# yhz0/SQLP

Hardware: AMD Instinct MI355X
Metric: stage-2 subproblems/sec + cut-gen HBM GB/s on STORM (higher is better)
Workload: dtype f64

## Files before the change

include/twosd_hip.h:

```cpp
#ifndef TWOSD_HIP_H
#define TWOSD_HIP_H

#include <stdint.h>

#ifdef __cplusplus
extern "C" {
#endif

typedef struct twosd_ctx twosd_ctx;

enum {
    TWOSD_OK = 0,
    TWOSD_E_ARG = -1,
    TWOSD_E_DEVICE = -2,
    TWOSD_E_STATE = -3,
    TWOSD_E_LP = -4,
    TWOSD_E_UNSUPPORTED = -5
};

enum { TWOSD_LP_OPTIMAL = 0, TWOSD_LP_INFEASIBLE = 1, TWOSD_LP_ITER_LIMIT = 2, TWOSD_LP_NUMERIC = 3 };

const char *twosd_last_error(void);

const char *twosd_version(void);
// ... 14 lines not shown
                         int index_base, int *m_lp, int *n_lp, int *n_bound_rows, int64_t *out_colptr,
                         int64_t *out_rowval, double *out_nzval, double *out_q, double *out_r, char *out_sense,
                         double *c0, int *col_src, double *col_sign, double *col_off, int *col_src2, int *box_col);

int twosd_set_random_positions(twosd_ctx *ctx, int k, const int *row, const int *col, int index_base);

int twosd_compute_basis(twosd_ctx *ctx, const double *x, const double *values);
int twosd_set_basis(twosd_ctx *ctx, const int *head);
int twosd_get_basis(twosd_ctx *ctx, int *head);

int twosd_pool_add_basis(twosd_ctx *ctx, const int *head, int *added);
int twosd_pool_build(twosd_ctx *ctx, int epi, const double *x, int first, int count, int max_pool,
                     int *pool_size);
int twosd_pool_build_candidates(twosd_ctx *ctx, int epi, const double *x, int first, int count, int level1,
                                int ncand);
int twosd_pool_refresh(twosd_ctx *ctx, int epi, const double *x, int first, int count, int max_pool,
                       int *pool_size);
int twosd_last_refresh_ms(twosd_ctx *ctx, double *ms5);

int twosd_refresh_train(twosd_ctx *ctx, int epi, const double *x, int first, int count, int *n_bases, double *box_lo,
                        double *box_hi);
int twosd_refresh_train_ex(twosd_ctx *ctx, int epi, const double *x, int first, int count, int kcap, int *n_bases,
                           int *n_optimal, double *box_lo, double *box_hi);
int twosd_refresh_cap_stats(twosd_ctx *ctx, int64_t *pivots_sum, int64_t *scenarios);
int twosd_training_cap(twosd_ctx *ctx, int64_t pivots_sum, int64_t scenarios, int *cap);
int twosd_select_refresh_bases(const uint64_t *keys, const int64_t *counts, const int64_t *reps, const int32_t *rank_of,
                               int n, int max_pool, int64_t *owner, int64_t *rep, int *npick);
int twosd_refresh_train_bases(twosd_ctx *ctx, uint64_t *keys, int *counts, int *reps);
int twosd_refresh_build_local(twosd_ctx *ctx, int n_own, const int *reps, int64_t *pack_bytes);
int twosd_refresh_pack(twosd_ctx *ctx, void *d_dst);
// ... 210 lines not shown
```

sqlp_amd/_lib.py:

```python
from __future__ import annotations

import ctypes as C
import os

_HERE = os.path.dirname(os.path.abspath(__file__))
LIB_PATH = os.path.join(_HERE, f"libtwosd_hip_{os.environ['TWOSD_LIB']}.so" if os.environ.get("TWOSD_LIB")
                        else "libtwosd_hip.so")

TWOSD_OK = 0
ERRORS = {-1: "TWOSD_E_ARG", -2: "TWOSD_E_DEVICE", -3: "TWOSD_E_STATE", -4: "TWOSD_E_LP",
          -5: "TWOSD_E_UNSUPPORTED"}
LP_OPTIMAL, LP_INFEASIBLE, LP_ITER_LIMIT, LP_NUMERIC = 0, 1, 2, 3

P = C.c_void_p
I = C.c_int
D = C.c_double
SIGNATURES = [
    ("twosd_last_error", C.c_char_p, []),
    ("twosd_version", C.c_char_p, []),
    ("twosd_create", I, [I, P]),
    ("twosd_destroy", I, [P]),
    ("twosd_set_template", I, [P, I, I, I, P, P, P, P, P, P, P, P, P, P, P, I]),
    ("twosd_lp_shape", I, [P, P, P, P]),
    ("twosd_canonical_form", I, [I, I, P, P, P, P, P, P, P, P, I, P, P, P, P, P, P, P, P, P, P, P, P, P, P, P]),
    ("twosd_set_random_positions", I, [P, I, P, P, I]),
    ("twosd_compute_basis", I, [P, P, P]),
    ("twosd_set_basis", I, [P, P]),
    ("twosd_get_basis", I, [P, P]),
    ("twosd_pool_add_basis", I, [P, P, P]),
    ("twosd_pool_build", I, [P, I, P, I, I, I, P]),
    ("twosd_pool_build_candidates", I, [P, I, P, I, I, I, I]),
    ("twosd_pool_refresh", I, [P, I, P, I, I, I, P]),
    ("twosd_last_refresh_ms", I, [P, P]),
    ("twosd_pool_size", I, [P, P]),
    ("twosd_pool_get", I, [P, I, P]),
    ("twosd_last_pool_picks", I, [P, I, P]),
    ("twosd_invalidate_x", I, [P]),
    ("twosd_epigraph_create", I, [P, P]),
    ("twosd_add_scenarios", I, [P, I, I, P, P]),
    ("twosd_epigraph_info", I, [P, I, P, P]),
    ("twosd_set_distributions", I, [P, I, P, P, P, P, P, P]),
    ("twosd_add_sampled_scenarios", I, [P, I, I, C.c_uint64, C.c_uint64, P]),
    ("twosd_get_scenarios", I, [P, I, I, I, P]),
    ("twosd_evaluate_sampled", I, [P, P, C.c_int64, C.c_int64, C.c_int64, C.c_uint64, P]),
    ("twosd_moments_merge", I, [P, P, P]),
    ("twosd_moments_of_values", I, [P, C.c_int64, P, P, P]),
# ... 142 lines not shown
```

sqlp_amd/csrc/lp_hyper.hip:

```cpp
#include <hip/hip_runtime.h>
#include <math.h>
#include <type_traits>
#include "twosd_internal.h"
#include "wave_ops.h"

namespace twosd {

#define HTOL_P 1e-9
#define HTOL_D 1e-9
#define HTOL_PIV 1e-9
#define HPI_ZERO 1e-12


#ifdef TWOSD_STAMPS
#define STAMP_DECL unsigned long long st_acc[10] = {0, 0, 0, 0, 0, 0, 0, 0, 0, 0}; \
    unsigned long long st_last = __builtin_amdgcn_s_memtime();
#define STAMP(i)                                                      \
    {                                                                 \
        const unsigned long long t_ = __builtin_amdgcn_s_memtime();   \
        st_acc[i] += t_ - st_last;                                    \
        st_last = t_;                                                 \
    }
#define STAMP_FLUSH                                                                         \
    if (lane == 0 && P.stamps)                                                              \
// ... 1035 lines not shown
    const int wid = __builtin_amdgcn_readfirstlane(threadIdx.x >> 6);
    const int s0 = blockIdx.x * kSelTile;
    const int ns = min(kSelTile, S.N - s0);
    const int sent = h_sel_sentinel(S.k);
    h_stage_sentinel(dvt, S.k);
    h_stage_pairs(dvt, S.dv, S.kcoef, S.k, ns, [&](int sl) { return s0 + sl; });
    if (threadIdx.x < kSelTile) sbest[threadIdx.x] = 0x7f800000u;
    __syncthreads();
    sel_f2 best = {INFINITY, INFINITY};
    int bpx = 0, bpy = 0;
    auto alive2 = [&](sel_f2 inf) {
        const float ox = __uint_as_float(__hip_atomic_load(&sbest[lane], __ATOMIC_RELAXED, __HIP_MEMORY_SCOPE_WORKGROUP));
        const float oy = __uint_as_float(__hip_atomic_load(&sbest[64 + lane], __ATOMIC_RELAXED, __HIP_MEMORY_SCOPE_WORKGROUP));
        return (inf.x < best.x && inf.x <= ox) || (inf.y < best.y && inf.y <= oy);
    };
    const int p_lo = (int)((long long)S.npool * blockIdx.y / gridDim.y), p_hi = (int)((long long)S.npool * (blockIdx.y + 1) / gridDim.y);
    bpx = bpy = p_lo;
    for (int p = p_lo + wid; p < p_hi; p += kSelWaves) {
        const sel_f2 inf = h_stream2(S.rec, S.sptr[p], S.send[p], S.cinf[p], S.cw, dvt2, sent, lane, alive2);
        if (inf.x < best.x) {
            best.x = inf.x;
            bpx = p;
            atomicMin(&sbest[lane], __float_as_uint(inf.x));
        }
        if (inf.y < best.y) {
            best.y = inf.y;
            bpy = p;
            atomicMin(&sbest[64 + lane], __float_as_uint(inf.y));
        }
    }
    bsum[wid][lane] = best.x; bidx[wid][lane] = bpx;
// ... 88 lines not shown
                const int cw = rci[w][sl];
                if (v < bk || (v == bk && cw >= 0 && (bc < 0 ? false : cw < bc))) { bk = v; bc = cw; }
            }
            const int s = S.order[t0 + sl];
            if (gridDim.y > 1) {
                S.pkey[(size_t)blockIdx.y * S.N + s] = bk;
                S.pci[(size_t)blockIdx.y * S.N + s] = bc;
            } else if (bc >= 0) {
                S.pick[s] = S.cand[(size_t)S.pick[s] * S.ncand + bc];
            }
        }
    }
}

__global__ void pool_select_merge_kernel(int N, int G, const float *__restrict__ pkey, const int *__restrict__ ppick, int *pick,
                                         float *key) {
    const int s = blockIdx.x * blockDim.x + threadIdx.x;
    if (s >= N) return;
    float b = pkey[s];
    int bp = ppick[s];
    for (int y = 1; y < G; ++y) {
        const float v = pkey[(size_t)y * N + s];
        const int p = ppick[(size_t)y * N + s];
        if (v < b || (v == b && p < bp)) { b = v; bp = p; }
    }
    pick[s] = bp;
    if (key) key[s] = b;
}
__global__ void pool_refine_merge_kernel(int N, int G, int ncand, const float *__restrict__ pkey, const int *__restrict__ pci,
                                         const int *__restrict__ cand, int *pick) {
    const int s = blockIdx.x * blockDim.x + threadIdx.x;
    if (s >= N) return;
    float bk = pkey[s];
    int bc = pci[s];
    for (int y = 1; y < G; ++y) {
        const float v = pkey[(size_t)y * N + s];
        const int c = pci[(size_t)y * N + s];
        if (v < bk || (v == bk && c >= 0 && (bc < 0 ? false : c < bc))) { bk = v; bc = c; }
    }
    if (bc >= 0) pick[s] = cand[(size_t)pick[s] * ncand + bc];
}

static int sel_split(int N, int items) {
    if (getenv("TWOSD_SEL_NOSPLIT")) return 1;
    const int nb = (N + kSelTile - 1) / kSelTile;
    int g = (1024 + nb - 1) / nb;
    g = std::min(g, std::max(1, items / kSelWaves));
    return std::max(1, std::min(g, 64));
}
int pool_select_split(int N, int npool) { return sel_split(N, npool); }
int pool_refine_split(int N, int ncand) { return sel_split(N, ncand); }

hipError_t launch_pool_refine(const PoolRefineParams &p, hipStream_t s) {
    if (p.N <= 0 || p.ncand <= 0) return hipSuccess;
    const int G = p.pkey ? pool_refine_split(p.N, p.ncand) : 1;
    hipLaunchKernelGGL(pool_refine_kernel, dim3((p.N + kSelTile - 1) / kSelTile, G), dim3(64 * kSelWaves), pool_select_lds_bytes(p.k), s, p);
    if (G > 1) hipLaunchKernelGGL(pool_refine_merge_kernel, dim3((p.N + 255) / 256), dim3(256), 0, s, p.N, G, p.ncand, p.pkey, p.pci, p.cand, p.pick);
    return hipGetLastError();
}

size_t pool_select_lds_bytes(int k) { return (size_t)4 * 65 * (kSelTile / 64) * (size_t)(std::max(k, 0) + 1); }

hipError_t launch_pool_select(const PoolSelParams &p, hipStream_t s) {
    if (p.N <= 0) return hipSuccess;
    const int nb = (p.N + kSelTile - 1) / kSelTile;
    const int G = p.pkey ? pool_select_split(p.N, p.npool) : 1;
    hipLaunchKernelGGL(pool_select_kernel, dim3(nb, G), dim3(64 * kSelWaves), pool_select_lds_bytes(p.k), s, p);
    if (G > 1) hipLaunchKernelGGL(pool_select_merge_kernel, dim3((p.N + 255) / 256), dim3(256), 0, s, p.N, G, p.pkey, p.ppick, p.pick, p.key);
    return hipGetLastError();
}

__global__ void __launch_bounds__(256) queue_records_kernel(int N, const int *__restrict__ order, const int *__restrict__ pick,
                                                           int2 *__restrict__ qrec) {
    const int q = blockIdx.x * blockDim.x + threadIdx.x;
    if (q >= N) return;
    const int s = order ? order[q] : q;
    qrec[q] = make_int2(s, pick ? pick[s] : 0);
}
hipError_t launch_queue_records(const int *order, const int *pick, int2 *qrec, int N, hipStream_t s) {
    if (N <= 0) return hipSuccess;
    hipLaunchKernelGGL(queue_records_kernel, dim3((N + 255) / 256), dim3(256), 0, s, N, order, pick, qrec);
    return hipGetLastError();
}
// ... 79 lines not shown
```

sqlp_amd/csrc/pool_refresh.hip:

```cpp
#include <hip/hip_runtime.h>
#include <algorithm>
#include <chrono>
#include <cmath>
#include <cstdio>
#include <cstdlib>
#include <cstring>
#include <vector>
#include "twosd_internal.h"
#include "twosd_ctx.h"

using namespace twosd;

using Clock = std::chrono::steady_clock;
static double ms_between(Clock::time_point a, Clock::time_point b) { return std::chrono::duration<double, std::milli>(b - a).count(); }


static const char *finish_composed(const twosd_ctx *c, PoolBasis &B) {
    const HostLP &L = c->L;
    pi0_from_rows(c, B);
    if (sparse_dual_infeasibility(L, B.head, B.pi0) > 1e-7) return "composed basis is not dual feasible";
    if (sparse_basis_residual(L, B.head, B.rptr, B.rcol, B.rval, 4) > 1e-8) return "composed B^{-1} inconsistent";
    return nullptr;
}

// ... 156 lines not shown
}

extern "C" int twosd_refresh_cap_stats(twosd_ctx *c, int64_t *pivots_sum, int64_t *scenarios) {
    if (!c) return fail(TWOSD_E_ARG, "refresh_cap_stats: NULL");
    if (pivots_sum) *pivots_sum = c->piv_ref_sum;
    if (scenarios) *scenarios = c->piv_ref_n;
    return TWOSD_OK;
}

extern "C" int twosd_set_refresh_kcap(twosd_ctx *c, int kcap) {
    if (!c) return fail(TWOSD_E_ARG, "set_refresh_kcap: NULL");
    c->train_kcap = kcap;
    return TWOSD_OK;
}

static int refresh_training(twosd_ctx *c, const double *x, const double *d_dv, int count, int kcap, bool retry, int *n_opt, bool dbg) {
    LpRun o;
    o.want_bkey = true;
    o.want_etas = true;
    o.want_head = true;
    o.kcap = kcap;
    int rc;
    if ((rc = run_lp(c, x, d_dv, count, o))) return rc;
    int opt = count;
    if (o.kcap > 0) {
        std::vector<int> st(count);
        HIPCHK(hipMemcpy(st.data(), c->d_status, sizeof(int) * count, hipMemcpyDeviceToHost));
        opt = (int)std::count(st.begin(), st.end(), (int)TWOSD_LP_OPTIMAL);
        if (retry && 2 * opt < count) {
            if (dbg) fprintf(stderr, "refresh training: %d of %d optimal under cap %d, solved again uncapped\n", opt, count, o.kcap);
            o.kcap = 0;
            if ((rc = run_lp(c, x, d_dv, count, o))) return rc;
        }
    }
    HIPCHK(hipStreamSynchronize(c->stream));
    unsigned long long used64 = 0;
    HIPCHK(hipMemcpy(&used64, c->d_eo_used, sizeof(used64), hipMemcpyDeviceToHost));
    if (used64 > c->eo_cap && used64 <= (unsigned long long)INT32_MAX) {
        if (dbg) fprintf(stderr, "refresh training: eta files of %llu entries past the arena of %zu, solved again\n", used64, c->eo_cap);
        c->eo_min_cap = (size_t)std::min<unsigned long long>(used64 + used64 / 8, INT32_MAX);
        if ((rc = run_lp(c, x, d_dv, count, o))) return rc;
    }
    c->last_train_opt = opt;
    if (n_opt) *n_opt = opt;
    return TWOSD_OK;
}

namespace {
struct RefreshFront {
    const EpiDevice *E = nullptr;
    const double *d_dv = nullptr;
    std::vector<int> reps, cnts;
// ... 36 lines not shown
        HIPCHK(hipMemcpy(F.reps.data(), d_list, sizeof(int) * U, hipMemcpyDeviceToHost));
        HIPCHK(hipMemcpy(F.cnts.data(), d_counts, sizeof(int) * U, hipMemcpyDeviceToHost));
    }
    F.t_bases = Clock::now();
    return TWOSD_OK;
}

extern "C" int twosd_pool_refresh(twosd_ctx *c, int epi, const double *x, int first, int count, int max_pool,
                                  int *pool_size) {
    const bool dbg = getenv("TWOSD_DEBUG") != nullptr;
    RefreshFront F;
    int rc;
    if ((rc = refresh_front(c, "pool_refresh", epi, x, first, count, max_pool >= 1, -1, true, nullptr, nullptr, dbg, F))) return rc;
    const int m = c->L.m, U = (int)F.reps.size();
    std::vector<int> ord(U);
    for (int a = 0; a < U; ++a) ord[a] = a;
    std::stable_sort(ord.begin(), ord.end(), [&](int a, int b) { return F.cnts[a] > F.cnts[b]; });
    const int R = std::min(U, max_pool - 1);
    std::vector<int> sel(R);
    for (int a = 0; a < R; ++a) sel[a] = F.reps[ord[a]];
    std::vector<PoolBasis> fresh;
    bool device_built = false;
    c->last_refresh_ms[1] = ms_between(F.t_trained, F.t_bases);
    c->last_refresh_ms[2] = c->last_refresh_ms[3] = 0.0;
    if (R > 0 && !getenv("TWOSD_REFRESH_HOST")) {
        if ((rc = c->d_refresh_sel.fit((size_t)R))) return rc;
        HIPCHK(hipMemcpyAsync(c->d_refresh_sel, sel.data(), sizeof(int) * R, hipMemcpyHostToDevice, c->stream));
        const int dev = refresh_build_device(c, R, dbg);
        if (dev < 0) return dev;
        device_built = dev == 0;
        c->last_refresh_ms[2] = ms_between(F.t_bases, Clock::now());
    }
// ... 336 lines not shown
```

sqlp_amd/csrc/pool_select.hip:

```cpp
#include <hip/hip_runtime.h>
#include <algorithm>
#include <cmath>
#include <cstdio>
#include <cstdlib>
#include <vector>
#include <chrono>
#include "twosd_internal.h"
#include "twosd_ctx.h"

using namespace twosd;

void twosd::reset_candidates(twosd_ctx *c) {
    c->pool_l1 = c->pool_ncand = 0;
    c->cand_pending = false;
    std::vector<int>().swap(c->cand_p1);
    std::vector<int>().swap(c->cand_pf);
}

int twosd::reserve_selection(twosd_ctx *c, int P, int records) {
    int rc;
    if ((rc = c->d_sel_code.fit(2 * (size_t)std::max(records, 1)))) return rc;
    if ((rc = c->d_sel_end.reserve((size_t)P)) || (rc = c->d_sel_cinf.reserve((size_t)P))) return rc;
    c->sel_cap_total = records;
    return TWOSD_OK;
// ... 316 lines not shown
            for (int p = 0; p < P; ++p) c->sel_nnz += end[p] - beg[p];
        }
    }
    c->prep_x.assign(x, x + n1);
    c->prep_valid = true;
    if (getenv("TWOSD_DEBUG")) {
        HIPCHK(hipStreamSynchronize(c->stream));
        fprintf(stderr, "prepare_x: P=%d %.3f ms (%lld selection records)\n", P,
                std::chrono::duration<double, std::milli>(std::chrono::steady_clock::now() - t_start).count(),
                (long long)c->sel_nnz);
    }
    return TWOSD_OK;
}

static int set_candidates(twosd_ctx *c, int level1, int ncand, int n, const int *p1, const int *pf) {
    std::vector<int> start(level1 + 1, 0);
    for (int s = 0; s < n; ++s)
        if (pf[s] != p1[s] && p1[s] >= 0 && p1[s] < level1) ++start[p1[s] + 1];
    for (int p = 0; p < level1; ++p) start[p + 1] += start[p];
    std::vector<int> fill(start.begin(), start.end() - 1), bucket(start[level1]);
    for (int s = 0; s < n; ++s)
        if (pf[s] != p1[s] && p1[s] >= 0 && p1[s] < level1) bucket[fill[p1[s]]++] = pf[s];
    std::vector<int> cand((size_t)level1 * ncand, -1);
    std::vector<std::pair<int, int>> v;
    for (int p = 0; p < level1; ++p) {
        int *b0 = bucket.data() + start[p], *b1 = bucket.data() + start[p + 1];
        if (b0 == b1) continue;
        std::sort(b0, b1);
        v.clear();
        for (int *a = b0; a < b1;) {
            int *b = a;
            while (b < b1 && *b == *a) ++b;
            v.push_back({-(int)(b - a), *a});
            a = b;
        }
        const size_t nk = std::min<size_t>(v.size(), ncand);
        std::partial_sort(v.begin(), v.begin() + nk, v.end());
        for (size_t i = 0; i < nk; ++i) cand[(size_t)p * ncand + i] = v[i].second;
    }
    if (getenv("TWOSD_DEBUG")) {
        int diff = 0, filled = 0;
        for (int s = 0; s < n; ++s) diff += pf[s] != p1[s];
        for (int v : cand) filled += v >= 0;
        fprintf(stderr, "pool candidates: P=%zu level1=%d: %d of %d training picks change, %d candidate slots filled\n",
                c->bp.bases.size(), level1, diff, n, filled);
    }
    int rc;
    int *h = c->stage[STG_CAND].reserve<int>(cand.size());
    if (!h) return fail(TWOSD_E_DEVICE, "pool candidates: pinned staging allocation failed");
    std::copy(cand.begin(), cand.end(), h);
    if ((rc = c->d_cand.reserve(cand.size()))) return rc;
    HIPCHK(hipMemcpyAsync(c->d_cand, h, sizeof(int) * cand.size(), hipMemcpyHostToDevice, c->stream));
    c->pool_l1 = level1;
    c->pool_ncand = ncand;
    c->cand_pending = false;
    return TWOSD_OK;
}

int twosd::select_pool(twosd_ctx *c, const double *d_dv, int N, int *d_pick, int npool_override) {
    const int P = (int)c->bp.bases.size();
    const bool two = npool_override <= 0 && c->pool_l1 > 0 && c->pool_l1 < P && c->pool_ncand > 0 && (c->d_cand || c->cand_pending);
    const int np1 = npool_override > 0 ? npool_override : two ? c->pool_l1 : P;
    int rc;
    size_t tb = 0, tb2 = 0;
    HIPCHK(sort_by_pool(d_pick, nullptr, N, P, nullptr, &tb, c->stream));
    HIPCHK(sort_by_pool(d_pick, nullptr, N, np1, nullptr, &tb2, c->stream));
    tb = std::max(tb, tb2);
    if ((size_t)N > c->d_order.cap || tb > c->d_sort_tmp.cap) {
        if ((rc = c->d_order.alloc((size_t)N)) || (rc = c->d_sort_tmp.alloc(tb))) return rc;
    }
    if (two && (rc = c->d_sel_key.fit((size_t)N))) return rc;
    const int g1 = pool_select_split(N, np1), g2 = two ? pool_refine_split(N, c->pool_ncand) : 1;
    const size_t pneed = (size_t)std::max(g1, g2) * N;
    if (std::max(g1, g2) > 1 && ((rc = c->d_sel_pkey.fit(pneed)) || (rc = c->d_sel_ppick.fit(pneed)))) return rc;
    PoolSelParams S{};
    S.N = N; S.k = c->k; S.npool = np1; S.dv = d_dv;
    S.kcoef = c->d_kcoef;
    S.cinf = c->d_sel_cinf; S.sptr = c->d_sel_ptr; S.send = c->d_sel_end; S.rec = reinterpret_cast<const int2 *>(c->d_sel_code.p);
    S.pick = d_pick;
    S.cw = c->sel_cw;
    S.key = two ? c->d_sel_key : nullptr;
    S.pkey = g1 > 1 ? c->d_sel_pkey : nullptr;
    S.ppick = g1 > 1 ? c->d_sel_ppick : nullptr;
    HIPCHK(launch_pool_select(S, c->stream));
    if (two && c->cand_pending &&
        (rc = set_candidates(c, c->cand_pl1, c->cand_pnc, (int)c->cand_p1.size(), c->cand_p1.data(), c->cand_pf.data())))
        return rc;
    if (two) {
        HIPCHK(sort_by_pool(d_pick, c->d_order, N, np1, c->d_sort_tmp, &tb, c->stream));
        PoolRefineParams Q{};
        Q.N = N; Q.k = c->k; Q.ncand = c->pool_ncand; Q.dv = d_dv; Q.kcoef = c->d_kcoef;
        Q.cinf = c->d_sel_cinf; Q.sptr = c->d_sel_ptr; Q.send = c->d_sel_end; Q.rec = S.rec;
        Q.order = c->d_order; Q.cand = c->d_cand; Q.pick = d_pick; Q.key = c->d_sel_key; Q.cw = c->sel_cw;
        Q.pkey = g2 > 1 ? c->d_sel_pkey : nullptr;
        Q.pci = g2 > 1 ? c->d_sel_ppick : nullptr;
        HIPCHK(launch_pool_refine(Q, c->stream));
    }
    HIPCHK(sort_by_pool(d_pick, c->d_order, N, P, c->d_sort_tmp, &tb, c->stream));
    return TWOSD_OK;
}

static int candidate_picks(twosd_ctx *c, const EpiDevice &E, const double *x, int first, int count, int level1,
                           int *p1, int *pf) {
    int rc;
    if ((rc = prepare_x(c, x))) return rc;
    if ((rc = c->d_cpick.reserve((size_t)count))) return rc;
    int *d_p = c->d_cpick;
    const double *dv = E.d_dv + (size_t)first * c->k;
    auto picks = [&](int np, int *out) {
        int r = select_pool(c, dv, count, d_p, np);
        if (!r && (hipStreamSynchronize(c->stream) != hipSuccess ||
                   hipMemcpy(out, d_p, sizeof(int) * count, hipMemcpyDeviceToHost) != hipSuccess))
            r = fail(TWOSD_E_DEVICE, "pool candidates: selection failed");
        return r;
    };
    rc = picks(level1, p1);
    if (!rc) rc = picks((int)c->bp.bases.size(), pf);
    return rc;
}

static int defer_candidates(twosd_ctx *c, int level1, int ncand, std::vector<int> &&p1, std::vector<int> &&pf) {
    c->cand_p1 = std::move(p1);
    c->cand_pf = std::move(pf);
    c->cand_pl1 = level1;
    c->cand_pnc = ncand;
    c->cand_pending = true;
    c->pool_l1 = level1;
    c->pool_ncand = ncand;
    return TWOSD_OK;
}

extern "C" int twosd_pool_candidate_picks(twosd_ctx *c, int epi, const double *x, int first, int count, int level1, int *p1,
                                          int *pf) {
    if (!c || !c->bp.has_basis) return fail(TWOSD_E_STATE, "pool_candidate_picks: no primary basis");
    if (epi < 0 || epi >= (int)c->epis.size()) return fail(TWOSD_E_ARG, "pool_candidate_picks: epigraph %d does not exist", epi);
    const EpiDevice &E = c->epis[epi];
    const int P = (int)c->bp.bases.size();
    if (first < 0 || count < 1 || first + count > E.count || level1 < 1 || level1 >= P || !p1 || !pf || (c->n1 > 0 && !x) ||
        c->CH <= 0)
        return fail(TWOSD_E_ARG, "pool_candidate_picks: bad arguments");
    HIPCHK(hipSetDevice(c->device));
    reset_candidates(c);
    return candidate_picks(c, E, x, first, count, level1, p1, pf);
}

extern "C" int twosd_pool_set_candidates(twosd_ctx *c, int level1, int ncand, int n, const int *p1, const int *pf) {
    if (!c || !c->bp.has_basis) return fail(TWOSD_E_STATE, "pool_set_candidates: no primary basis");
    const int P = (int)c->bp.bases.size();
    if (level1 < 1 || level1 >= P || ncand < 1 || ncand > 1024 || n < 0 || (n > 0 && (!p1 || !pf)))
        return fail(TWOSD_E_ARG, "pool_set_candidates: bad arguments");
    for (int s = 0; s < n; ++s)
        if (p1[s] < 0 || p1[s] >= P || pf[s] < 0 || pf[s] >= P) return fail(TWOSD_E_ARG, "pool_set_candidates: pick outside the pool");
    HIPCHK(hipSetDevice(c->device));
    return defer_candidates(c, level1, ncand, std::vector<int>(p1, p1 + n), std::vector<int>(pf, pf + n));
}

extern "C" int twosd_pool_build_candidates(twosd_ctx *c, int epi, const double *x, int first, int count, int level1,
                                           int ncand) {
    if (!c || !c->bp.has_basis) return fail(TWOSD_E_STATE, "pool_build_candidates: no primary basis");
    if (epi < 0 || epi >= (int)c->epis.size()) return fail(TWOSD_E_ARG, "pool_build_candidates: epigraph %d does not exist", epi);
    const EpiDevice &E = c->epis[epi];
    const int P = (int)c->bp.bases.size();
    if (first < 0 || count < 1 || first + count > E.count || level1 < 0 || ncand < 0 || ncand > 1024 || (c->n1 > 0 && !x))
        return fail(TWOSD_E_ARG, "pool_build_candidates: bad arguments");
    reset_candidates(c);
    if (level1 == 0 || ncand == 0 || level1 >= P || P < 2 || c->CH <= 0) return TWOSD_OK;
    HIPCHK(hipSetDevice(c->device));
    std::vector<int> p1(count), pf(count);
    int rc;
    if ((rc = candidate_picks(c, E, x, first, count, level1, p1.data(), pf.data()))) return rc;
    return defer_candidates(c, level1, ncand, std::move(p1), std::move(pf));
}

extern "C" int twosd_last_pool_picks(twosd_ctx *c, int N, int *picks) {
    if (!c || !picks || N < 0 || N > c->last.N) return fail(TWOSD_E_ARG, "last_pool_picks: bad arguments");
    if (c->bp.bases.size() <= 1 || !c->d_pool_pick) {
        std::fill(picks, picks + N, 0);
        return TWOSD_OK;
    }
    HIPCHK(hipMemcpy(picks, c->d_pool_pick, sizeof(int) * N, hipMemcpyDeviceToHost));
    return TWOSD_OK;
}

extern "C" int twosd_invalidate_x(twosd_ctx *c) {
    if (!c) return fail(TWOSD_E_ARG, "invalidate_x: NULL context");
    c->prep_valid = false;
// ... 3 lines not shown
```

sqlp_amd/csrc/twosd_ctx.h:

```cpp
#pragma once
#include <hip/hip_runtime.h>
#include <stdint.h>
#include <algorithm>
#include <memory>
#include <thread>
#include <vector>
#include "devbuf.h"
#include "twosd_internal.h"
#include "basis_pool.h"

#define HIPCHK(expr)                                                                                      \
    do {                                                                                                  \
        hipError_t _e = (expr);                                                                           \
        if (_e != hipSuccess) return twosd::fail(TWOSD_E_DEVICE, "%s: %s", #expr, hipGetErrorString(_e)); \
    } while (0)

namespace twosd {

enum StageSlot : int {
    STG_POOL_RCOL = 0, STG_POOL_CROW, STG_POOL_RVAL, STG_POOL_CVAL, STG_POOL_D0,
    STG_ELEM_KE, STG_ELEM_KIX, STG_ELEM_KRAW, STG_ELEM_KV,
    STG_PG_TOT,
    STG_FREE_10,
    STG_PG_NZ,
    STG_PG_IOFF,
    STG_RT_SEG,
    STG_RT_HDR,
    STG_CAND,
    STG_COUNT
};
static_assert(STG_PG_TOT == 9 && STG_CAND == 15 && STG_COUNT == 16, "a slot keeps its buffer: do not renumber");

struct BoxCache {
    int epi = -1, first = -1, count = -1, n = -1;
    bool operator==(const BoxCache &o) const { return epi == o.epi && first == o.first && count == o.count && n == o.n; }
};

struct EpiDevice {
// ... 190 lines not shown
    std::unique_ptr<twosd::CutWs, void (*)(twosd::CutWs *)> cut_ws{nullptr, twosd::cut_free};
    int last_cut_epi = -1, last_cut_n = 0, last_cut_nv = 0;
    twosd::ReformState reform;
    std::unique_ptr<twosd::VkeyWs, void (*)(twosd::VkeyWs *)> vkey_ws{nullptr, twosd::vkey_free};
    twosd::DevBuf<unsigned long long> d_vkey, d_bkey;
    twosd::DevBuf<int> d_eo_pb, d_eo_K, d_eo_off, d_eo_etap, d_eo_etaoff;
    twosd::DevBuf<int> d_eo_eidx;
    twosd::DevBuf<unsigned long long> d_eo_used;
    twosd::DevBuf<double> d_eo_evals;
    size_t eo_rows = 0;
    size_t eo_cap = 0;
    size_t eo_min_cap = 0;
    int eo_kmax = 0;
    double last_refresh_ms[5] = {0, 0, 0, 0, 0};
    twosd::DevBuf<int> d_refresh_sel;
    twosd::BoxCache sel_box;
    twosd::DevBuf<double> d_pg_amax, d_pg_d0p, d_pg_ival;
    twosd::DevBuf<int> d_pg_irow;
    twosd::DevBuf<long long> d_pg_ioff;
    twosd::DevBuf<int> d_pg_cnt, d_pg_tot, d_pg_valid, d_pg_head0;
    twosd::DevBuf<int> d_pg_map, d_pg_off, d_pg_pos;
    twosd::DevBuf<int> d_pg_scrow, d_pg_scoff;
    twosd::DevBuf<double> d_pg_scval;
    long long pg_sc_cap = 0;
    std::vector<unsigned long long> rt_keys;
    std::vector<int> rt_counts, rt_reps;
    std::vector<double> rt_lo, rt_hi;
    twosd::BoxCache rt_box;
    int rt_nown = -1;
    bool rt_trained = false;
// ... 36 lines not shown
    bool want_etas = false;
    bool want_head = false;
    const int *d_list = nullptr;
    int nlist = 0;
    int kcap = 0;
    double *lp_us_out = nullptr;
    bool want_ray = false;
};
int run_lp(twosd_ctx *c, const double *x, const double *d_dv, int N, const LpRun &o = LpRun());
#pragma GCC visibility push(hidden)
double template_value(const twosd_ctx *c, int e);
void rhs_at(const twosd_ctx *c, const double *x, const double *dv, std::vector<double> &b);
SampleParams sample_params(const twosd_ctx *c, int n, uint64_t seed, uint64_t first_index, double *out);
int draw_scenarios(twosd_ctx *c, int n, uint64_t seed, uint64_t first_index, double *out, int mode, int G);
int upload_lintr(twosd_ctx *c, const LintrTables &T);
int select_pool(twosd_ctx *c, const double *d_dv, int N, int *d_pick, int npool_override);
int copy_lp_outputs(twosd_ctx *c, int N, double *obj, double *pi, double *y, int *status, const double *d_w);
int prepare_elements(twosd_ctx *c);
int reserve_selection(twosd_ctx *c, int P, int records);
void reset_candidates(twosd_ctx *c);
int training_box(twosd_ctx *c, const EpiDevice &E, int epi, int first, int count, std::vector<double> &lo,
                 std::vector<double> &hi, BoxCache *cache);
#pragma GCC visibility pop
template <typename F>
void parallel_for(int n, F f, int serial_below = 64) {
    const int nth = (int)std::max(1u, std::min(16u, std::thread::hardware_concurrency()));
    if (n < serial_below || nth == 1) {
        for (int i = 0; i < n; ++i) f(i);
        return;
    }
    std::vector<std::thread> th;
// ... 24 lines not shown
```

sqlp_amd/csrc/twosd_internal.h:

```cpp
#pragma once
#include <hip/hip_runtime.h>
#include <stdint.h>
#include <string>
#include <vector>
#include "twosd_hip.h"
#include "devbuf.h"
#include "dist_tables.h"
#include "lintr_tables.h"
#include "pool_pack.h"

namespace twosd {

constexpr int kWave = 64;
constexpr int kWavesPerBlock = 4;
constexpr int kMaxColsPerLane = 64;

enum : int { BT_Y = 0, BT_G = 1, BT_L = 2, BT_E = 3 };


constexpr int kQueueStride = 32;
constexpr int kMaxQueueGroups = 64;
struct HyperParams {
    int m, n, k, N, kmax, ecap;
    int kcap;
// ... 98 lines not shown
    z = (z ^ (z >> 27)) * 0x94D049BB133111EBull;
    return z ^ (z >> 31);
}

struct PoolSelParams {
    int N, k, npool;
    const double *dv;
    const double *kcoef;
    const float *cinf;
    const int *sptr, *send;
    const int2 *rec;
    int *pick;
    float cw;
    float *key;
    float *pkey; int *ppick;
};
struct PoolRefineParams {
    int N, k, ncand;
    const double *dv, *kcoef;
    const float *cinf;
    const int *sptr, *send;
    const int2 *rec;
    const int *order, *cand;
    int *pick;
    const float *key;
    float cw;
    float *pkey; int *pci;
};
hipError_t launch_pool_refine(const PoolRefineParams &p, hipStream_t s);
size_t pool_select_lds_bytes(int k);
int pool_select_split(int N, int npool);
int pool_refine_split(int N, int ncand);
hipError_t sort_by_pool(const int *pick, int *order, int N, int npool, void *tmp, size_t *tmp_bytes, hipStream_t s);
hipError_t launch_pool_select(const PoolSelParams &p, hipStream_t s);
size_t hyper_lds_bytes(int R, int C, int kmax, int k);
int hyper_rows_per_lane(int m);
int hyper_cols_per_lane(int ncols);
hipError_t launch_hyper(int R, int C, const HyperParams &p, int nblocks, size_t lds, hipStream_t s);
hipError_t launch_queue_records(const int *order, const int *pick, int2 *qrec, int N, hipStream_t s);
int hyper_max_blocks_per_cu(int R, int C, int kmax, int k);


struct SampleParams {
    int N, k;
    unsigned long long seed, first_index;
    const int *kind;
    const int *off;
// ... 49 lines not shown
```

sqlp_amd/twosd.py:

```python
from __future__ import annotations

import ctypes as C
from dataclasses import dataclass, field
from typing import Optional

import numpy as np

from . import _lib
from ._lib import check, ptr
from .smps import spStageProblem, spSmpsPosition, scenario_positions, sto_positions

MIN_SENSE = "MIN_SENSE"
DEFAULT_TIE_REL = 0.0


def _f64(a):
    return np.ascontiguousarray(a, dtype=np.float64)


@dataclass
class CanonicalForm:
    m_lp: int
    n_lp: int
    n_bound_rows: int
# ... 141 lines not shown
        head = np.ascontiguousarray(head, dtype=np.int32)
        added = C.c_int(0)
        check(self.lib.twosd_pool_add_basis(self.h, ptr(head), C.byref(added)))
        return bool(added.value)

    def pool_build(self, epi, x, first, count, max_pool) -> int:
        x = _f64(x)
        n = C.c_int(0)
        check(self.lib.twosd_pool_build(self.h, epi.index, ptr(x), int(first), int(count), int(max_pool),
                                        C.byref(n)))
        return n.value

    def pool_build_candidates(self, epi, x, first, count, level1, ncand):
        check(self.lib.twosd_pool_build_candidates(self.h, epi.index, ptr(_f64(x)), int(first), int(count),
                                                   int(level1), int(ncand)))

    def last_pool_picks(self, N):
        picks = np.zeros(N, dtype=np.int32)
        check(self.lib.twosd_last_pool_picks(self.h, int(N), ptr(picks)))
        return picks

    def invalidate_x(self):
        check(self.lib.twosd_invalidate_x(self.h))

    def pool_refresh(self, epi, x, first, count, max_pool) -> int:
        n = C.c_int()
        check(self.lib.twosd_pool_refresh(self.h, epi.index, ptr(_f64(x)), first, count, max_pool, C.byref(n)))
        return n.value

    def refresh_train(self, epi, x, first, count):
# ... 1066 lines not shown
```

Before: 18.26 million.

## Build pool candidate lists on device and fuse level-1 and full selection

Computes the level-1 and full-pool picks in one select launch by splitting the grid's y-blocks between the two pool ranges, with the merge kernel recording the level-1 best. A new kernel then builds the per-basis candidate lists on the GPU with LDS histograms and a bitonic sort, so the picks no longer round-trip to the host. Refresh training counts optimal statuses in a small device kernel and reads back one pinned pair instead of copying the whole status array, and a stable sort is replaced by a counting sort. It also adds a query API for the candidate lists; the device path is limited by pool and width caps, and ties may order differently than on the host.

```diff
diff --git a/include/twosd_hip.h b/include/twosd_hip.h
--- a/include/twosd_hip.h
+++ b/include/twosd_hip.h
@@ -52,6 +52,7 @@
                      int *pool_size);
 int twosd_pool_build_candidates(twosd_ctx *ctx, int epi, const double *x, int first, int count, int level1,
                                 int ncand);
+int twosd_pool_candidates(twosd_ctx *ctx, int *level1, int *ncand, int *out);
 int twosd_pool_refresh(twosd_ctx *ctx, int epi, const double *x, int first, int count, int max_pool,
                        int *pool_size);
 int twosd_last_refresh_ms(twosd_ctx *ctx, double *ms5);
diff --git a/sqlp_amd/_lib.py b/sqlp_amd/_lib.py
--- a/sqlp_amd/_lib.py
+++ b/sqlp_amd/_lib.py
@@ -30,6 +30,7 @@
     ("twosd_pool_add_basis", I, [P, P, P]),
     ("twosd_pool_build", I, [P, I, P, I, I, I, P]),
     ("twosd_pool_build_candidates", I, [P, I, P, I, I, I, I]),
+    ("twosd_pool_candidates", I, [P, P, P, P]),
     ("twosd_pool_refresh", I, [P, I, P, I, I, I, P]),
     ("twosd_last_refresh_ms", I, [P, P]),
     ("twosd_pool_size", I, [P, P]),
diff --git a/sqlp_amd/csrc/cand_lists.h b/sqlp_amd/csrc/cand_lists.h
--- /dev/null
+++ b/sqlp_amd/csrc/cand_lists.h
@@ -0,0 +1,50 @@
+#pragma once
+#include <algorithm>
+#include <cstddef>
+#include <utility>
+#include <vector>
+
+namespace twosd {
+
+constexpr int kCandBasisBits = 13;
+constexpr int kCandBasisMask = (1 << kCandBasisBits) - 1;
+constexpr int kCandMaxPool = 1 << kCandBasisBits;
+constexpr int kCandMaxCount = (1 << (32 - kCandBasisBits)) - 1;
+constexpr int kCandMaxWidth = 1024;
+constexpr unsigned cand_pack(unsigned count, int basis) {
+    return count ? (count << kCandBasisBits) | (unsigned)(kCandBasisMask - basis) : 0u;
+}
+constexpr int cand_unpack(unsigned key) { return key ? kCandBasisMask - (int)(key & (unsigned)kCandBasisMask) : -1; }
+constexpr bool cand_device_limits(int npool, int ncand, int n) {
+    return npool <= kCandMaxPool && ncand <= kCandMaxWidth && n <= kCandMaxCount;
+}
+
+inline void cand_lists_host(int level1, int ncand, int n, const int *p1, const int *pf, std::vector<int> &cand) {
+    cand.assign((size_t)level1 * ncand, -1);
+    auto counted = [&](int s) { return pf[s] != p1[s] && p1[s] >= 0 && p1[s] < level1; };
+    std::vector<int> start(level1 + 1, 0);
+    for (int s = 0; s < n; ++s)
+        if (counted(s)) ++start[p1[s] + 1];
+    for (int p = 0; p < level1; ++p) start[p + 1] += start[p];
+    std::vector<int> fill(start.begin(), start.end() - 1), bucket(start[level1]);
+    for (int s = 0; s < n; ++s)
+        if (counted(s)) bucket[fill[p1[s]]++] = pf[s];
+    std::vector<std::pair<int, int>> v;
+    for (int p = 0; p < level1; ++p) {
+        int *b0 = bucket.data() + start[p], *b1 = bucket.data() + start[p + 1];
+        if (b0 == b1) continue;
+        std::sort(b0, b1);
+        v.clear();
+        for (int *a = b0; a < b1;) {
+            int *b = a;
+            while (b < b1 && *b == *a) ++b;
+            v.push_back({-(int)(b - a), *a});
+            a = b;
+        }
+        const size_t nk = std::min<size_t>(v.size(), (size_t)ncand);
+        std::partial_sort(v.begin(), v.begin() + nk, v.end());
+        for (size_t i = 0; i < nk; ++i) cand[(size_t)p * ncand + i] = v[i].second;
+    }
+}
+
+}
diff --git a/sqlp_amd/csrc/lp_hyper.hip b/sqlp_amd/csrc/lp_hyper.hip
--- a/sqlp_amd/csrc/lp_hyper.hip
+++ b/sqlp_amd/csrc/lp_hyper.hip
@@ -1073,7 +1073,15 @@
         const float oy = __uint_as_float(__hip_atomic_load(&sbest[64 + lane], __ATOMIC_RELAXED, __HIP_MEMORY_SCOPE_WORKGROUP));
         return (inf.x < best.x && inf.x <= ox) || (inf.y < best.y && inf.y <= oy);
     };
-    const int p_lo = (int)((long long)S.npool * blockIdx.y / gridDim.y), p_hi = (int)((long long)S.npool * (blockIdx.y + 1) / gridDim.y);
+    int r0 = 0, rn = S.npool, cy = blockIdx.y, cn = gridDim.y;
+    if (S.pick1) {
+        const bool low = cy < S.G1;
+        r0 = low ? 0 : S.L;
+        rn = low ? S.L : S.npool - S.L;
+        cn = low ? S.G1 : cn - S.G1;
+        cy = low ? cy : cy - S.G1;
+    }
+    const int p_lo = r0 + (int)((long long)rn * cy / cn), p_hi = r0 + (int)((long long)rn * (cy + 1) / cn);
     bpx = bpy = p_lo;
     for (int p = p_lo + wid; p < p_hi; p += kSelWaves) {
         const sel_f2 inf = h_stream2(S.rec, S.sptr[p], S.send[p], S.cinf[p], S.cw, dvt2, sent, lane, alive2);
@@ -1192,15 +1200,17 @@
 }
 
 __global__ void pool_select_merge_kernel(int N, int G, const float *__restrict__ pkey, const int *__restrict__ ppick, int *pick,
-                                         float *key) {
+                                         float *key, int G1, int *pick1) {
     const int s = blockIdx.x * blockDim.x + threadIdx.x;
     if (s >= N) return;
     float b = pkey[s];
     int bp = ppick[s];
+    if (pick1 && G1 == 1) pick1[s] = bp;
     for (int y = 1; y < G; ++y) {
         const float v = pkey[(size_t)y * N + s];
         const int p = ppick[(size_t)y * N + s];
         if (v < b || (v == b && p < bp)) { b = v; bp = p; }
+        if (pick1 && y + 1 == G1) pick1[s] = bp;
     }
     pick[s] = bp;
     if (key) key[s] = b;
@@ -1227,6 +1237,11 @@
     return std::max(1, std::min(g, 64));
 }
 int pool_select_split(int N, int npool) { return sel_split(N, npool); }
+void pool_select_split2(int N, int L, int npool, int *g1, int *g2) {
+    const int g = sel_split(N, npool);
+    *g1 = std::max(1, std::min((int)(((long long)g * L + npool / 2) / npool), L / kSelWaves));
+    *g2 = std::max(1, std::min(g - *g1, (npool - L) / kSelWaves));
+}
 int pool_refine_split(int N, int ncand) { return sel_split(N, ncand); }
 
 hipError_t launch_pool_refine(const PoolRefineParams &p, hipStream_t s) {
@@ -1242,9 +1257,17 @@
 hipError_t launch_pool_select(const PoolSelParams &p, hipStream_t s) {
     if (p.N <= 0) return hipSuccess;
     const int nb = (p.N + kSelTile - 1) / kSelTile;
-    const int G = p.pkey ? pool_select_split(p.N, p.npool) : 1;
-    hipLaunchKernelGGL(pool_select_kernel, dim3(nb, G), dim3(64 * kSelWaves), pool_select_lds_bytes(p.k), s, p);
-    if (G > 1) hipLaunchKernelGGL(pool_select_merge_kernel, dim3((p.N + 255) / 256), dim3(256), 0, s, p.N, G, p.pkey, p.ppick, p.pick, p.key);
+    int G = p.pkey ? pool_select_split(p.N, p.npool) : 1, G1 = 0;
+    PoolSelParams q = p;
+    if (p.pick1) {
+        if (!p.pkey || !p.ppick || p.L <= 0 || p.L >= p.npool) return hipErrorInvalidValue;
+        int G2;
+        pool_select_split2(p.N, p.L, p.npool, &G1, &G2);
+        G = G1 + G2;
+    }
+    q.G1 = G1;
+    hipLaunchKernelGGL(pool_select_kernel, dim3(nb, G), dim3(64 * kSelWaves), pool_select_lds_bytes(p.k), s, q);
+    if (G > 1) hipLaunchKernelGGL(pool_select_merge_kernel, dim3((p.N + 255) / 256), dim3(256), 0, s, p.N, G, p.pkey, p.ppick, p.pick, p.key, G1, p.pick1);
     return hipGetLastError();
 }
 
diff --git a/sqlp_amd/csrc/pool_refresh.hip b/sqlp_amd/csrc/pool_refresh.hip
--- a/sqlp_amd/csrc/pool_refresh.hip
+++ b/sqlp_amd/csrc/pool_refresh.hip
@@ -194,6 +194,23 @@
     return TWOSD_OK;
 }
 
+constexpr int kTallyThreads = 1024;
+__global__ void __launch_bounds__(kTallyThreads) refresh_tally_kernel(int n, const int *__restrict__ status,
+                                                                      const unsigned long long *__restrict__ eo_used,
+                                                                      unsigned long long *__restrict__ out) {
+    __shared__ int total;
+    if (threadIdx.x == 0) total = 0;
+    __syncthreads();
+    int mine = 0;
+    for (int s = threadIdx.x; s < n; s += kTallyThreads) mine += status[s] == TWOSD_LP_OPTIMAL;
+    if (mine) atomicAdd(&total, mine);
+    __syncthreads();
+    if (threadIdx.x == 0) {
+        out[0] = (unsigned long long)total;
+        out[1] = *eo_used;
+    }
+}
+
 static int refresh_training(twosd_ctx *c, const double *x, const double *d_dv, int count, int kcap, bool retry, int *n_opt, bool dbg) {
     LpRun o;
     o.want_bkey = true;
@@ -202,20 +219,28 @@
     o.kcap = kcap;
     int rc;
     if ((rc = run_lp(c, x, d_dv, count, o))) return rc;
+    if ((rc = c->d_train_tally.reserve(2))) return rc;
+    unsigned long long *h_tally = c->stage[STG_TRAIN_TALLY].reserve<unsigned long long>(2);
+    if (!h_tally) return fail(TWOSD_E_DEVICE, "pool refresh: pinned staging allocation failed");
+    auto tally = [&]() -> int {
+        hipLaunchKernelGGL(refresh_tally_kernel, dim3(1), dim3(kTallyThreads), 0, c->stream, count, c->d_status.p, c->d_eo_used.p,
+                           c->d_train_tally.p);
+        HIPCHK(hipGetLastError());
+        HIPCHK(hipMemcpyAsync(h_tally, c->d_train_tally, 2 * sizeof(unsigned long long), hipMemcpyDeviceToHost, c->stream));
+        HIPCHK(hipStreamSynchronize(c->stream));
+        return TWOSD_OK;
+    };
+    if ((rc = tally())) return rc;
     int opt = count;
     if (o.kcap > 0) {
-        std::vector<int> st(count);
-        HIPCHK(hipMemcpy(st.data(), c->d_status, sizeof(int) * count, hipMemcpyDeviceToHost));
-        opt = (int)std::count(st.begin(), st.end(), (int)TWOSD_LP_OPTIMAL);
+        opt = (int)h_tally[0];
         if (retry && 2 * opt < count) {
             if (dbg) fprintf(stderr, "refresh training: %d of %d optimal under cap %d, solved again uncapped\n", opt, count, o.kcap);
             o.kcap = 0;
-            if ((rc = run_lp(c, x, d_dv, count, o))) return rc;
+            if ((rc = run_lp(c, x, d_dv, count, o)) || (rc = tally())) return rc;
         }
     }
-    HIPCHK(hipStreamSynchronize(c->stream));
-    unsigned long long used64 = 0;
-    HIPCHK(hipMemcpy(&used64, c->d_eo_used, sizeof(used64), hipMemcpyDeviceToHost));
+    const unsigned long long used64 = h_tally[1];
     if (used64 > c->eo_cap && used64 <= (unsigned long long)INT32_MAX) {
         if (dbg) fprintf(stderr, "refresh training: eta files of %llu entries past the arena of %zu, solved again\n", used64, c->eo_cap);
         c->eo_min_cap = (size_t)std::min<unsigned long long>(used64 + used64 / 8, INT32_MAX);
@@ -282,8 +307,12 @@
     if ((rc = refresh_front(c, "pool_refresh", epi, x, first, count, max_pool >= 1, -1, true, nullptr, nullptr, dbg, F))) return rc;
     const int m = c->L.m, U = (int)F.reps.size();
     std::vector<int> ord(U);
-    for (int a = 0; a < U; ++a) ord[a] = a;
-    std::stable_sort(ord.begin(), ord.end(), [&](int a, int b) { return F.cnts[a] > F.cnts[b]; });
+    int cmax = 0;
+    for (int a = 0; a < U; ++a) cmax = std::max(cmax, F.cnts[a]);
+    std::vector<int> at((size_t)cmax + 2, 0);
+    for (int a = 0; a < U; ++a) ++at[cmax - std::max(F.cnts[a], 0) + 1];
+    for (int i = 0; i <= cmax; ++i) at[i + 1] += at[i];
+    for (int a = 0; a < U; ++a) ord[at[cmax - std::max(F.cnts[a], 0)]++] = a;
     const int R = std::min(U, max_pool - 1);
     std::vector<int> sel(R);
     for (int a = 0; a < R; ++a) sel[a] = F.reps[ord[a]];
diff --git a/sqlp_amd/csrc/pool_select.hip b/sqlp_amd/csrc/pool_select.hip
--- a/sqlp_amd/csrc/pool_select.hip
+++ b/sqlp_amd/csrc/pool_select.hip
@@ -7,6 +7,7 @@
 #include <chrono>
 #include "twosd_internal.h"
 #include "twosd_ctx.h"
+#include "cand_lists.h"
 
 using namespace twosd;
 
@@ -354,30 +355,8 @@
 }
 
 static int set_candidates(twosd_ctx *c, int level1, int ncand, int n, const int *p1, const int *pf) {
-    std::vector<int> start(level1 + 1, 0);
-    for (int s = 0; s < n; ++s)
-        if (pf[s] != p1[s] && p1[s] >= 0 && p1[s] < level1) ++start[p1[s] + 1];
-    for (int p = 0; p < level1; ++p) start[p + 1] += start[p];
-    std::vector<int> fill(start.begin(), start.end() - 1), bucket(start[level1]);
-    for (int s = 0; s < n; ++s)
-        if (pf[s] != p1[s] && p1[s] >= 0 && p1[s] < level1) bucket[fill[p1[s]]++] = pf[s];
-    std::vector<int> cand((size_t)level1 * ncand, -1);
-    std::vector<std::pair<int, int>> v;
-    for (int p = 0; p < level1; ++p) {
-        int *b0 = bucket.data() + start[p], *b1 = bucket.data() + start[p + 1];
-        if (b0 == b1) continue;
-        std::sort(b0, b1);
-        v.clear();
-        for (int *a = b0; a < b1;) {
-            int *b = a;
-            while (b < b1 && *b == *a) ++b;
-            v.push_back({-(int)(b - a), *a});
-            a = b;
-        }
-        const size_t nk = std::min<size_t>(v.size(), ncand);
-        std::partial_sort(v.begin(), v.begin() + nk, v.end());
-        for (size_t i = 0; i < nk; ++i) cand[(size_t)p * ncand + i] = v[i].second;
-    }
+    std::vector<int> cand;
+    cand_lists_host(level1, ncand, n, p1, pf, cand);
     if (getenv("TWOSD_DEBUG")) {
         int diff = 0, filled = 0;
         for (int s = 0; s < n; ++s) diff += pf[s] != p1[s];
@@ -397,11 +376,73 @@
     return TWOSD_OK;
 }
 
-int twosd::select_pool(twosd_ctx *c, const double *d_dv, int N, int *d_pick, int npool_override) {
+constexpr int kCandThreads = 1024;
+__global__ void __launch_bounds__(kCandThreads) cand_lists_kernel(int n, int P, int ncand, const int *__restrict__ p1,
+                                                                  const int *__restrict__ pf, int *__restrict__ cand) {
+    __shared__ unsigned key[kCandMaxPool];
+    __shared__ int any;
+    const int p = blockIdx.x, tid = threadIdx.x;
+    int psort = 2;
+    while (psort < P) psort <<= 1;
+    for (int i = tid; i < psort; i += kCandThreads) key[i] = 0u;
+    if (tid == 0) any = 0;
+    __syncthreads();
+    bool mine = false;
+    for (int s = tid; s < n; s += kCandThreads) {
+        const int f = pf[s];
+        if (p1[s] == p && f != p && (unsigned)f < (unsigned)P) {
+            atomicAdd(&key[f], 1u);
+            mine = true;
+        }
+    }
+    if (mine) any = 1;
+    __syncthreads();
+    int *row = cand + (size_t)p * ncand;
+    if (!any) {
+        for (int i = tid; i < ncand; i += kCandThreads) row[i] = -1;
+        return;
+    }
+    for (int i = tid; i < psort; i += kCandThreads) key[i] = cand_pack(key[i], i);
+    __syncthreads();
+    for (int kk = 2; kk <= psort; kk <<= 1) {
+        for (int j = kk >> 1; j > 0; j >>= 1) {
+            for (int t = tid; t < psort / 2; t += kCandThreads) {
+                const int a = 2 * j * (t / j) + (t % j), b = a + j;
+                const bool down = (a & kk) == 0;
+                const unsigned ka = key[a], kb = key[b];
+                if ((ka < kb) == down) {
+                    key[a] = kb;
+                    key[b] = ka;
+                }
+            }
+            __syncthreads();
+        }
+    }
+    for (int i = tid; i < ncand; i += kCandThreads) row[i] = i < psort ? cand_unpack(key[i]) : -1;
+}
+
+int twosd::select_pool(twosd_ctx *c, const double *d_dv, int N, int *d_pick, int level1, int *d_pick1) {
     const int P = (int)c->bp.bases.size();
-    const bool two = npool_override <= 0 && c->pool_l1 > 0 && c->pool_l1 < P && c->pool_ncand > 0 && (c->d_cand || c->cand_pending);
-    const int np1 = npool_override > 0 ? npool_override : two ? c->pool_l1 : P;
-    int rc;
+    int rc;
+    PoolSelParams S{};
+    S.N = N; S.k = c->k; S.npool = P; S.dv = d_dv;
+    S.kcoef = c->d_kcoef;
+    S.cinf = c->d_sel_cinf; S.sptr = c->d_sel_ptr; S.send = c->d_sel_end; S.rec = reinterpret_cast<const int2 *>(c->d_sel_code.p);
+    S.pick = d_pick;
+    S.cw = c->sel_cw;
+    if (d_pick1) {
+        if (level1 <= 0 || level1 >= P) return fail(TWOSD_E_ARG, "pool selection: boundary %d outside the pool of %d", level1, P);
+        int ga, gb;
+        pool_select_split2(N, level1, P, &ga, &gb);
+        const size_t pneed = (size_t)(ga + gb) * N;
+        if ((rc = c->d_sel_pkey.fit(pneed)) || (rc = c->d_sel_ppick.fit(pneed))) return rc;
+        S.pkey = c->d_sel_pkey; S.ppick = c->d_sel_ppick;
+        S.L = level1; S.pick1 = d_pick1;
+        HIPCHK(launch_pool_select(S, c->stream));
+        return TWOSD_OK;
+    }
+    const bool two = c->pool_l1 > 0 && c->pool_l1 < P && c->pool_ncand > 0 && (c->d_cand || c->cand_pending);
+    const int np1 = two ? c->pool_l1 : P;
     size_t tb = 0, tb2 = 0;
     HIPCHK(sort_by_pool(d_pick, nullptr, N, P, nullptr, &tb, c->stream));
     HIPCHK(sort_by_pool(d_pick, nullptr, N, np1, nullptr, &tb2, c->stream));
@@ -413,12 +454,7 @@
     const int g1 = pool_select_split(N, np1), g2 = two ? pool_refine_split(N, c->pool_ncand) : 1;
     const size_t pneed = (size_t)std::max(g1, g2) * N;
     if (std::max(g1, g2) > 1 && ((rc = c->d_sel_pkey.fit(pneed)) || (rc = c->d_sel_ppick.fit(pneed)))) return rc;
-    PoolSelParams S{};
-    S.N = N; S.k = c->k; S.npool = np1; S.dv = d_dv;
-    S.kcoef = c->d_kcoef;
-    S.cinf = c->d_sel_cinf; S.sptr = c->d_sel_ptr; S.send = c->d_sel_end; S.rec = reinterpret_cast<const int2 *>(c->d_sel_code.p);
-    S.pick = d_pick;
-    S.cw = c->sel_cw;
+    S.npool = np1;
     S.key = two ? c->d_sel_key : nullptr;
     S.pkey = g1 > 1 ? c->d_sel_pkey : nullptr;
     S.ppick = g1 > 1 ? c->d_sel_ppick : nullptr;
@@ -440,23 +476,18 @@
     return TWOSD_OK;
 }
 
-static int candidate_picks(twosd_ctx *c, const EpiDevice &E, const double *x, int first, int count, int level1,
-                           int *p1, int *pf) {
+static int candidate_picks(twosd_ctx *c, const EpiDevice &E, const double *x, int first, int count, int level1) {
     int rc;
     if ((rc = prepare_x(c, x))) return rc;
-    if ((rc = c->d_cpick.reserve((size_t)count))) return rc;
-    int *d_p = c->d_cpick;
-    const double *dv = E.d_dv + (size_t)first * c->k;
-    auto picks = [&](int np, int *out) {
-        int r = select_pool(c, dv, count, d_p, np);
-        if (!r && (hipStreamSynchronize(c->stream) != hipSuccess ||
-                   hipMemcpy(out, d_p, sizeof(int) * count, hipMemcpyDeviceToHost) != hipSuccess))
-            r = fail(TWOSD_E_DEVICE, "pool candidates: selection failed");
-        return r;
-    };
-    rc = picks(level1, p1);
-    if (!rc) rc = picks((int)c->bp.bases.size(), pf);
-    return rc;
+    if ((rc = c->d_cpick.reserve(2 * (size_t)count))) return rc;
+    return select_pool(c, E.d_dv + (size_t)first * c->k, count, c->d_cpick + count, level1, c->d_cpick);
+}
+static int candidate_picks_host(twosd_ctx *c, int count, int *p1, int *pf) {
+    if (hipMemcpyAsync(p1, c->d_cpick, sizeof(int) * count, hipMemcpyDeviceToHost, c->stream) != hipSuccess ||
+        hipMemcpyAsync(pf, c->d_cpick + count, sizeof(int) * count, hipMemcpyDeviceToHost, c->stream) != hipSuccess ||
+        hipStreamSynchronize(c->stream) != hipSuccess)
+        return fail(TWOSD_E_DEVICE, "pool candidates: selection failed");
+    return TWOSD_OK;
 }
 
 static int defer_candidates(twosd_ctx *c, int level1, int ncand, std::vector<int> &&p1, std::vector<int> &&pf) {
@@ -481,7 +512,8 @@
         return fail(TWOSD_E_ARG, "pool_candidate_picks: bad arguments");
     HIPCHK(hipSetDevice(c->device));
     reset_candidates(c);
-    return candidate_picks(c, E, x, first, count, level1, p1, pf);
+    if (int rc = candidate_picks(c, E, x, first, count, level1)) return rc;
+    return candidate_picks_host(c, count, p1, pf);
 }
 
 extern "C" int twosd_pool_set_candidates(twosd_ctx *c, int level1, int ncand, int n, const int *p1, const int *pf) {
@@ -506,10 +538,38 @@
     reset_candidates(c);
     if (level1 == 0 || ncand == 0 || level1 >= P || P < 2 || c->CH <= 0) return TWOSD_OK;
     HIPCHK(hipSetDevice(c->device));
-    std::vector<int> p1(count), pf(count);
-    int rc;
-    if ((rc = candidate_picks(c, E, x, first, count, level1, p1.data(), pf.data()))) return rc;
-    return defer_candidates(c, level1, ncand, std::move(p1), std::move(pf));
+    int rc;
+    if ((rc = candidate_picks(c, E, x, first, count, level1))) return rc;
+    const char *host = getenv("TWOSD_CAND_HOST");
+    if ((host && atoi(host) != 0) || !cand_device_limits(P, ncand, count)) {
+        std::vector<int> p1(count), pf(count);
+        if ((rc = candidate_picks_host(c, count, p1.data(), pf.data()))) return rc;
+        return defer_candidates(c, level1, ncand, std::move(p1), std::move(pf));
+    }
+    if ((rc = c->d_cand.reserve((size_t)level1 * ncand))) return rc;
+    hipLaunchKernelGGL(cand_lists_kernel, dim3(level1), dim3(kCandThreads), 0, c->stream, count, P, ncand, c->d_cpick.p,
+                       c->d_cpick + count, c->d_cand.p);
+    HIPCHK(hipGetLastError());
+    c->pool_l1 = level1;
+    c->pool_ncand = ncand;
+    return TWOSD_OK;
+}
+
+extern "C" int twosd_pool_candidates(twosd_ctx *c, int *level1, int *ncand, int *out) {
+    if (!c || !level1 || !ncand) return fail(TWOSD_E_ARG, "pool_candidates: NULL");
+    HIPCHK(hipSetDevice(c->device));
+    int rc;
+    if (c->cand_pending &&
+        (rc = set_candidates(c, c->cand_pl1, c->cand_pnc, (int)c->cand_p1.size(), c->cand_p1.data(), c->cand_pf.data())))
+        return rc;
+    const bool have = c->pool_l1 > 0 && c->pool_ncand > 0 && c->d_cand;
+    *level1 = have ? c->pool_l1 : 0;
+    *ncand = have ? c->pool_ncand : 0;
+    if (have && out) {
+        HIPCHK(hipMemcpyAsync(out, c->d_cand, sizeof(int) * (size_t)c->pool_l1 * c->pool_ncand, hipMemcpyDeviceToHost, c->stream));
+        HIPCHK(hipStreamSynchronize(c->stream));
+    }
+    return TWOSD_OK;
 }
 
 extern "C" int twosd_last_pool_picks(twosd_ctx *c, int N, int *picks) {
diff --git a/sqlp_amd/csrc/twosd_ctx.h b/sqlp_amd/csrc/twosd_ctx.h
--- a/sqlp_amd/csrc/twosd_ctx.h
+++ b/sqlp_amd/csrc/twosd_ctx.h
@@ -21,7 +21,7 @@
     STG_POOL_RCOL = 0, STG_POOL_CROW, STG_POOL_RVAL, STG_POOL_CVAL, STG_POOL_D0,
     STG_ELEM_KE, STG_ELEM_KIX, STG_ELEM_KRAW, STG_ELEM_KV,
     STG_PG_TOT,
-    STG_FREE_10,
+    STG_TRAIN_TALLY,
     STG_PG_NZ,
     STG_PG_IOFF,
     STG_RT_SEG,
@@ -242,6 +242,7 @@
     int eo_kmax = 0;
     double last_refresh_ms[5] = {0, 0, 0, 0, 0};
     twosd::DevBuf<int> d_refresh_sel;
+    twosd::DevBuf<unsigned long long> d_train_tally;
     twosd::BoxCache sel_box;
     twosd::DevBuf<double> d_pg_amax, d_pg_d0p, d_pg_ival;
     twosd::DevBuf<int> d_pg_irow;
@@ -308,7 +309,7 @@
 SampleParams sample_params(const twosd_ctx *c, int n, uint64_t seed, uint64_t first_index, double *out);
 int draw_scenarios(twosd_ctx *c, int n, uint64_t seed, uint64_t first_index, double *out, int mode, int G);
 int upload_lintr(twosd_ctx *c, const LintrTables &T);
-int select_pool(twosd_ctx *c, const double *d_dv, int N, int *d_pick, int npool_override);
+int select_pool(twosd_ctx *c, const double *d_dv, int N, int *d_pick, int level1 = 0, int *d_pick1 = nullptr);
 int copy_lp_outputs(twosd_ctx *c, int N, double *obj, double *pi, double *y, int *status, const double *d_w);
 int prepare_elements(twosd_ctx *c);
 int reserve_selection(twosd_ctx *c, int P, int records);
diff --git a/sqlp_amd/csrc/twosd_internal.h b/sqlp_amd/csrc/twosd_internal.h
--- a/sqlp_amd/csrc/twosd_internal.h
+++ b/sqlp_amd/csrc/twosd_internal.h
@@ -136,6 +136,8 @@
     float cw;
     float *key;
     float *pkey; int *ppick;
+    int L, G1;
+    int *pick1;
 };
 struct PoolRefineParams {
     int N, k, ncand;
@@ -153,6 +155,7 @@
 size_t pool_select_lds_bytes(int k);
 int pool_select_split(int N, int npool);
 int pool_refine_split(int N, int ncand);
+void pool_select_split2(int N, int L, int npool, int *g1, int *g2);
 hipError_t sort_by_pool(const int *pick, int *order, int N, int npool, void *tmp, size_t *tmp_bytes, hipStream_t s);
 hipError_t launch_pool_select(const PoolSelParams &p, hipStream_t s);
 size_t hyper_lds_bytes(int R, int C, int kmax, int k);
diff --git a/sqlp_amd/twosd.py b/sqlp_amd/twosd.py
--- a/sqlp_amd/twosd.py
+++ b/sqlp_amd/twosd.py
@@ -179,6 +179,14 @@
     def pool_build_candidates(self, epi, x, first, count, level1, ncand):
         check(self.lib.twosd_pool_build_candidates(self.h, epi.index, ptr(_f64(x)), int(first), int(count),
                                                    int(level1), int(ncand)))
+
+    def pool_candidates(self):
+        l1, nc = C.c_int(), C.c_int()
+        check(self.lib.twosd_pool_candidates(self.h, C.byref(l1), C.byref(nc), None))
+        out = np.zeros((l1.value, nc.value), dtype=np.int32)
+        if out.size:
+            check(self.lib.twosd_pool_candidates(self.h, C.byref(l1), C.byref(nc), ptr(out)))
+        return l1.value, nc.value, out
 
     def last_pool_picks(self, N):
         picks = np.zeros(N, dtype=np.int32)
```

Result: no change. 18.39 million, median of 6 (+0.7%).
